# vitskvara/VBMatrixFactorization.jl

Hardware: AMD Instinct MI355X
Metric: VB iterations/sec (higher is better)
Workload: dtype bf16

## Files before the change

vbmatrixfactorization.jl_amd/csrc/gram_kernels.hpp:

```cpp
#pragma once
#include "common.hpp"
#include "ctrl_kernels.hpp"
#include "post_kernels.hpp"

namespace vbmf {

#ifndef GRAM_CHUNK
#define GRAM_CHUNK 256
#endif
constexpr int GRAM_PLANES = 5;
constexpr long long GRAM_G_NT_BYTES = 240LL << 20;

__device__ __forceinline__ unsigned pack_bf2(unsigned short lo, unsigned short hi) { return (unsigned)lo | ((unsigned)hi << 16); }

__global__ __launch_bounds__(256) void gram_build_kernel(const uint4* __restrict__ Y1, int XT, int KS, float* __restrict__ Gt,
                                                         int GT) {
    const int P = blockIdx.y, Q = blockIdx.x;
    if (P > Q) return;
    const int lane = threadIdx.x & 63, w = threadIdx.x >> 6;
    const int p0 = 4 * P + 2 * (w >> 1), q0 = 4 * Q + 2 * (w & 1);
    const long long KT = 2LL * GT;
    double g64[2][2][16];
#pragma unroll
    for (int a = 0; a < 2; ++a)
// ... 155 lines not shown
    for (int mb = 0; mb < GW_KS; ++mb) {
        const long long m = row0 + 16 * mb + c;
        f64x4 acc = {0.0, 0.0, 0.0, 0.0};
#pragma unroll
        for (int s = 0; s < NS; ++s) {
            const float4 a = m < M ? *reinterpret_cast<const float4*>(A32 + m * HP + 16 * s + 4 * q) : make_float4(0.f, 0.f, 0.f, 0.f);
            acc = __builtin_amdgcn_mfma_f64_16x16x4f64((double)a.x, sb[s][0], acc, 0, 0, 0);
            acc = __builtin_amdgcn_mfma_f64_16x16x4f64((double)a.y, sb[s][1], acc, 0, 0, 0);
            acc = __builtin_amdgcn_mfma_f64_16x16x4f64((double)a.z, sb[s][2], acc, 0, 0, 0);
            acc = __builtin_amdgcn_mfma_f64_16x16x4f64((double)a.w, sb[s][3], acc, 0, 0, 0);
        }
#pragma unroll
        for (int r = 0; r < 4; ++r) sW[16 * mb + q + 4 * r][16 * cb + c] = (float)acc[r];
    }
    __syncthreads();
    const long long plane = (long long)KT * NH * 64;
    for (int it = threadIdx.x; it < GW_KS * NHC * 64; it += NT) {
        const int jj = it / (NHC * 64), htl = (it / 64) % NHC, ln = it & 63;
        const int half = ln >> 5, hl = 32 * htl + (ln & 31), h = col0 + hl, ht = blockIdx.y * NHC + htl;
        const long long j = (long long)blockIdx.x * GW_KS + jj;
        if (j >= KT) continue;
        unsigned short wp[3][8], dp[2][8];
#pragma unroll
        for (int e = 0; e < 8; ++e) {
            const long long m = 16 * j + 8 * half + e;
            const float wv = sW[16 * jj + 8 * half + e][hl];
            const float dv = (float)((double)wv - (double)Wold[m * HP + h]);
            Wnew[m * HP + h] = wv;
            wp[0][e] = f2bf(wv);
            float res = wv - bf2f(wp[0][e]);
            wp[1][e] = f2bf(res);
            res -= bf2f(wp[1][e]);
            wp[2][e] = f2bf(res);
            dp[0][e] = f2bf(dv);
            dp[1][e] = f2bf(dv - bf2f(dp[0][e]));
        }
        const long long o = (j * NH + ht) * 64 + ln;
#pragma unroll
        for (int p = 0; p < 3; ++p)
            Wt[p * plane + o] = make_uint4(pack_bf2(wp[p][0], wp[p][1]), pack_bf2(wp[p][2], wp[p][3]), pack_bf2(wp[p][4], wp[p][5]),
                                           pack_bf2(wp[p][6], wp[p][7]));
#pragma unroll
        for (int p = 0; p < 2; ++p)
            Wt[(3 + p) * plane + o] = make_uint4(pack_bf2(dp[p][0], dp[p][1]), pack_bf2(dp[p][2], dp[p][3]), pack_bf2(dp[p][4], dp[p][5]),
                                                 pack_bf2(dp[p][6], dp[p][7]));
    }
}

__device__ __forceinline__ float sub_f32(float a, float b) {
    float r;
    asm("v_sub_f32 %0, %1, %2" : "=v"(r) : "v"(a), "v"(b));
    return r;
}
__device__ __forceinline__ unsigned cvt_pk_bf16(float lo, float hi) {
    typedef __attribute__((ext_vector_type(2))) float f32x2v;
    typedef __attribute__((ext_vector_type(2))) __bf16 bf16x2v;
    const f32x2v v = {lo, hi};
    return __builtin_bit_cast(unsigned, __builtin_convertvector(v, bf16x2v));
}
__device__ __forceinline__ void split3_frag(const f32x4& x0, const f32x4& x1, u32x4v& g0, u32x4v& g1, u32x4v& g2) {
    const float v[8] = {x0.x, x0.y, x0.z, x0.w, x1.x, x1.y, x1.z, x1.w};
#pragma unroll
    for (int e = 0; e < 4; ++e) {
        float a = v[2 * e], b = v[2 * e + 1];
        const unsigned p0 = cvt_pk_bf16(a, b);
        a = sub_f32(a, bitsf(p0 << 16));
        b = sub_f32(b, bitsf(p0 & 0xffff0000u));
        const unsigned p1 = cvt_pk_bf16(a, b);
        a = sub_f32(a, bitsf(p1 << 16));
        b = sub_f32(b, bitsf(p1 & 0xffff0000u));
        g0[e] = p0;
        g1[e] = p1;
        g2[e] = cvt_pk_bf16(a, b);
    }
}

__device__ __forceinline__ f32x16 mfma_bf(const u32x4v& a, const u32x4v& b, const f32x16& c) {
    return __builtin_amdgcn_mfma_f32_32x32x16_bf16(__builtin_bit_cast(bf16x8, a), __builtin_bit_cast(bf16x8, b), c, 0, 0, 0);
}

#ifndef VBMF_GRAMPROD_PROBE
#define VBMF_GRAMPROD_PROBE 0
#endif
template <int NH>
struct GramProd {
    static constexpr int NW = 8;
    static constexpr int THREADS = 64 * NW;
    static constexpr int TPG = 16 / NH;
    static constexpr int NXW = TPG >= NW ? TPG / NW : 1;
    static constexpr int HS = TPG >= NW ? 1 : NW / TPG;
    static constexpr int NHW = NH / HS;
    static constexpr int CH = NH == 2 ? 4 : 2;
    static constexpr int D = 4;
    static constexpr int U = CH;
    static constexpr int NP = GRAM_PLANES * CH * NH;
    static constexpr int PPW = (NP + NW - 1) / NW;
    static constexpr int GL = 2 * NXW;
    static constexpr int GQ = VBMF_GRAMPROD_PROBE == 2 ? 0 : GL;
    static constexpr int PLANE_BYTES = 2 * NP * 1024;
    static constexpr int RING_BYTES = NW * D * GL * 1024;
    static constexpr int LDS_BYTES = PLANE_BYTES + RING_BYTES;
    static_assert(NXW * (NW / HS) == TPG && NHW * HS == NH, "gram_prod geometry");
    static_assert(LDS_BYTES <= 160 * 1024, "gram_prod LDS");
    static constexpr int g_wait(int u) {
        int n = (D - 1) * GQ;
        for (int d = 1; d < D; ++d) n += ((u + CH * D - d) % CH == 0) ? PPW : 0;
        return n;
    }
};
template <int NH, int NHT = NH>
__global__ __launch_bounds__(GramProd<NH>::THREADS) void gram_prod_kernel(const float4* __restrict__ Gt, const uint4* __restrict__ Wt,
                                                                          float* __restrict__ Out, int GT, int XT1, int sps, int nrg,
                                                                          long long n, long long slab_floats,
                                                                          const int* __restrict__ stop) {
    using C = GramProd<NH>;
    constexpr int NW = C::NW, NXW = C::NXW, NHW = C::NHW, D = C::D, CH = C::CH, U = C::U, NP = C::NP, PPW = C::PPW, GL = C::GL;
    extern __shared__ __attribute__((aligned(1024))) unsigned char gram_lds[];
    if (*stop) return;
    const int lane = threadIdx.x & 63;
    const int w = __builtin_amdgcn_readfirstlane(threadIdx.x >> 6);
    const int rg = blockIdx.x % nrg, s = blockIdx.x / nrg;
    const int KT = 2 * GT;
    const int j0 = s * sps, j1 = min(j0 + sps, KT), nk = j1 - j0;
    const int pt0 = rg * C::TPG + (w % (C::TPG / NXW)) * NXW;
    const int h0 = (w / (C::TPG / NXW)) * NHW;
    const int hg0 = NHT == NH ? 0 : (int)blockIdx.y * NH;
    const long long plane = (long long)KT * NHT * 64;
    f32x16 accP[NXW][NHW], accQ[NXW][NHW];
#pragma unroll
    for (int i = 0; i < NXW; ++i)
#pragma unroll
        for (int h = 0; h < NHW; ++h)
#pragma unroll
            for (int r = 0; r < 16; ++r) { accP[i][h][r] = 0.f; accQ[i][h][r] = 0.f; }
    __amdgpu_buffer_rsrc_t gr[NXW];
#pragma unroll
    for (int i = 0; i < NXW; ++i)
        gr[i] = __builtin_amdgcn_make_buffer_rsrc((void*)(Gt + (long long)(pt0 + i) * KT * 128), 0,
                                                  VBMF_GRAMPROD_PROBE == 1 ? 0u : (unsigned)KT * 2048u, 0x00020000);
    const __amdgpu_buffer_rsrc_t wr = __builtin_amdgcn_make_buffer_rsrc((void*)Wt, 0, (unsigned)(GRAM_PLANES * plane * 16), 0x00020000);
    const int voff = lane * 16;
    unsigned char* const ring = gram_lds + C::PLANE_BYTES + w * (D * GL * 1024);
    const bool g_nt = !(NH == 4 && NHT == 4) && (long long)GT * GT * 4096 > GRAM_G_NT_BYTES;
    auto load_g = [&](int slot, int t) __attribute__((always_inline)) {
        const int so = VBMF_GRAMPROD_PROBE == 3 ? 0 : min(j0 + t, j1 - 1) * 2048;
        if (g_nt) {
#pragma unroll
            for (int i = 0; i < NXW; ++i) {
                lds_dma_piece_nt(gr[i], ring + (slot * GL + 2 * i) * 1024, voff, so);
                lds_dma_piece_nt(gr[i], ring + (slot * GL + 2 * i + 1) * 1024, voff, so + 1024);
            }
        } else {
#pragma unroll
            for (int i = 0; i < NXW; ++i) {
                lds_dma_piece(gr[i], ring + (slot * GL + 2 * i) * 1024, voff, so);
                lds_dma_piece(gr[i], ring + (slot * GL + 2 * i + 1) * 1024, voff, so + 1024);
            }
        }
    };
    auto load_planes = [&](int cc, int t) __attribute__((always_inline)) {
#pragma unroll
        for (int v = 0; v < PPW; ++v) {
            const int x = min(w + NW * v, NP - 1);
            const int q = x / (CH * NH), r = x % (CH * NH);
            const int j = min(j0 + t + r / NH, j1 - 1);
            lds_dma_piece(wr, gram_lds + (cc * NP + x) * 1024, voff, (int)(q * plane + ((long long)j * NHT + hg0 + r % NH) * 64) * 16);
        }
    };
#pragma unroll
    for (int d = 0; d < D; ++d) {
        if ((d + CH * D - D) % CH == 0) load_planes(0, 0);
        load_g(d, d);
    }
    asm volatile("s_waitcnt vmcnt(%0)" ::"n"(CH * GL) : "memory");
    __builtin_amdgcn_s_barrier();
    asm volatile("" ::: "memory");
    u32x4v wf[GRAM_PLANES][NHW], g[NXW][3];
    auto mma = [&]() __attribute__((always_inline)) {
#pragma unroll
        for (int i = 0; i < NXW; ++i) {
#pragma unroll
            for (int h = 0; h < NHW; ++h) {
                f32x16 a = accP[i][h];
                a = mfma_bf(wf[2][h], g[i][0], a);
                a = mfma_bf(wf[1][h], g[i][1], a);
                a = mfma_bf(wf[0][h], g[i][2], a);
                a = mfma_bf(wf[1][h], g[i][0], a);
                a = mfma_bf(wf[0][h], g[i][1], a);
                accP[i][h] = mfma_bf(wf[0][h], g[i][0], a);
                f32x16 d = accQ[i][h];
                d = mfma_bf(wf[4][h], g[i][0], d);
                d = mfma_bf(wf[3][h], g[i][1], d);
                accQ[i][h] = mfma_bf(wf[3][h], g[i][0], d);
            }
        }
    };
    int slot = 0;
    auto body = [&](int t0, bool tail) __attribute__((always_inline)) {
#pragma unroll
        for (int u = 0; u < U; ++u) {
            const int t = t0 + u, kk = u % CH;
            const int cc = (t / CH) & 1;
            const bool live = !tail || t < nk;
            asm volatile("s_waitcnt vmcnt(%0)" ::"n"(C::g_wait(u)) : "memory");
            if (live) {
                const unsigned char* gs = ring + slot * (GL * 1024) + lane * 32;
                f32x4 x[NXW][2];
#pragma unroll
                for (int i = 0; i < NXW; ++i) {
                    x[i][0] = *reinterpret_cast<const f32x4*>(gs + i * 2048);
                    x[i][1] = *reinterpret_cast<const f32x4*>(gs + i * 2048 + 16);
                }
                const unsigned char* pl = gram_lds + (cc * NP + kk * NH + h0) * 1024 + lane * 16;
#pragma unroll
                for (int q = 0; q < GRAM_PLANES; ++q)
#pragma unroll
                    for (int h = 0; h < NHW; ++h) wf[q][h] = *reinterpret_cast<const u32x4v*>(pl + (q * CH * NH + h) * 1024);
#pragma unroll
                for (int i = 0; i < NXW; ++i) split3_frag(x[i][0], x[i][1], g[i][0], g[i][1], g[i][2]);
            }
            __builtin_amdgcn_sched_barrier(0);
            if (kk == 0) load_planes(cc ^ 1, t + CH);
            if (VBMF_GRAMPROD_PROBE != 2) load_g(slot, t + D);
            slot = slot + 1 == D ? 0 : slot + 1;
            __builtin_amdgcn_sched_barrier(0);
            if (live) mma();
            if (kk == CH - 1) {
                asm volatile("s_waitcnt vmcnt(%0) lgkmcnt(0)" ::"n"(CH * C::GQ) : "memory");
                __builtin_amdgcn_s_barrier();
                asm volatile("" ::: "memory");
            }
        }
    };
    int t0 = 0;
    for (; t0 + U <= nk; t0 += U) body(t0, false);
    if (t0 < nk) body(t0, true);
    asm volatile("s_waitcnt vmcnt(0)" ::: "memory");
    float4* oP = reinterpret_cast<float4*>(Out + (long long)s * slab_floats);
    float4* oQ = reinterpret_cast<float4*>(Out + (long long)s * slab_floats + n);
#pragma unroll
    for (int i = 0; i < NXW; ++i) {
        const int p = pt0 + i;
        if (p >= XT1) continue;
#pragma unroll
        for (int h = 0; h < NHW; ++h) {
            const long long o = (((long long)p * NHT + hg0 + h0 + h) * 64 + lane) * 4;
            const f32x16 a = accP[i][h], d = accQ[i][h];
#pragma unroll
            for (int q = 0; q < 4; ++q) {
                oP[o + q] = float4{a[4 * q], a[4 * q + 1], a[4 * q + 2], a[4 * q + 3]};
                oQ[o + q] = float4{d[4 * q], d[4 * q + 1], d[4 * q + 2], d[4 * q + 3]};
            }
        }
    }
}

template <int HP>
struct GPart {
    static constexpr int V = HP / 16, S = 8 / V, NH = HP / 32;
    static constexpr int NT = 512, SD = 8;
    static constexpr int PPT = HP == 128 ? 2 : 3;
    static constexpr int ROWS = PPT * NT * 4 / HP;
    static constexpr int NSTEP = ROWS / 4 / S;
    static constexpr int BUF = ROWS * HP;
    static constexpr int SU = V == 8 ? 2 : 4;
    static_assert(NSTEP % SU == 0 && (ROWS / 4) % S == 0 && ROWS % 16 == 0, "gram_tail geometry");
    static_assert((S - 1) * V * V * 64 * 32 <= 2 * BUF * 4, "gram_tail: the subset fold reuses the block buffers");
};
template <int HP>
__device__ __forceinline__ int gpart_index(int a, int b) {
    constexpr int V = GPart<HP>::V;
    const int tw = a % V, i = a / V, t = b % V, c = b / V;
    return ((((tw * V + t) * 4 + (i >> 2)) << 6) + 16 * (i & 3) + c);
}
__device__ __forceinline__ void add4(float4& s, const float4& v) { s.x += v.x; s.y += v.y; s.z += v.z; s.w += v.w; }
struct GTailRound { float4 a0, a1, a2, a3, a4, a5, a6, a7; };
__device__ __forceinline__ void gtail_load(GTailRound& v, const __amdgpu_buffer_rsrc_t (&r)[8], int voff, int cnt) {
    const auto ld = [&](int u) __attribute__((always_inline)) {
        return __builtin_bit_cast(float4, __builtin_amdgcn_raw_buffer_load_b128(r[u], voff, 0, 0));
    };
    switch (cnt) {
        default: v.a7 = ld(7); [[fallthrough]];
        case 7: v.a6 = ld(6); [[fallthrough]];
        case 6: v.a5 = ld(5); [[fallthrough]];
        case 5: v.a4 = ld(4); [[fallthrough]];
        case 4: v.a3 = ld(3); [[fallthrough]];
        case 3: v.a2 = ld(2); [[fallthrough]];
        case 2: v.a1 = ld(1); [[fallthrough]];
        case 1: v.a0 = ld(0);
    }
}
template <bool FIRST>
__device__ __forceinline__ float4 gtail_sum(const GTailRound& v, float4 f, int cnt) {
    if (FIRST) f = v.a0;
    else add4(f, v.a0);
    if (cnt > 1) add4(f, v.a1);
    if (cnt > 2) add4(f, v.a2);
    if (cnt > 3) add4(f, v.a3);
    if (cnt > 4) add4(f, v.a4);
    if (cnt > 5) add4(f, v.a5);
    if (cnt > 6) add4(f, v.a6);
    if (cnt > 7) add4(f, v.a7);
    return f;
}
template <int HP, int HPT>
struct GPartBlk {
    static constexpr int NQ = HPT / HP;
    static constexpr long long STRIDE = 2LL * HPT * HPT + (NQ == 1 ? 1 : NQ);
};
template <int HP, int HPT = HP>
__global__ __launch_bounds__(512) void gram_tail_kernel(const float* slabs, int nslab, long long slab_floats, float* PQ, long long n,
                                                        long long Mp1, const float* __restrict__ Wn, const float* __restrict__ Wo,
                                                        const float* __restrict__ A32, long long M, int rpc, int nchunk,
                                                        double* __restrict__ part, const int* __restrict__ stop) {
    using C = GPart<HP>;
    constexpr int V = C::V, S = C::S, NH = C::NH, PPT = C::PPT, SD = C::SD, ROWS = C::ROWS, NSTEP = C::NSTEP, SU = C::SU;
    constexpr int NQ = GPartBlk<HP, HPT>::NQ, NHT = HPT / 32;
    constexpr bool BLK = NQ > 1;
    constexpr long long STRIDE = GPartBlk<HP, HPT>::STRIDE;
// ... 215 lines not shown
```

vbmatrixfactorization.jl_amd/csrc/vbmf_hip.hip:

```cpp
#include "../../include/vbmf_hip.h"

#include <hip/hip_runtime.h>
#include <rccl/rccl.h>

#include <algorithm>
#include <chrono>
#include <cmath>
#include <cstdio>
#include <cstring>
#include <string>
#include <thread>
#include <type_traits>
#include <vector>

#include "common.hpp"
#include "ctx_cache.hpp"
#include "ctx_mem.hpp"
#include "ctrl_kernels.hpp"
#include "post_kernels.hpp"
#include "rng.hpp"
#include "sparse_kernels.hpp"
#include "stream_gemm.hpp"
#include "tile_kernels.hpp"
#include "prep_kernels.hpp"
// ... 767 lines not shown
        }
        TRY(side_join(c));
        if (fused_gram(c)) TRY(launch_post_gram(c, 0, c->Pred));
        else if (c->P_frag) TRY(launch_post_frag(c, 0, c->Pred));
        else TRY(launch_post(c, 0, c->Pred, 1));
    } else {
        TRY(side_join(c));
        if (fused_gram(c)) TRY(launch_post_gram(c, 0, c->P));
        else if (c->P_frag) TRY(launch_post_frag(c, 0, c->P));
        else TRY(launch_post(c, 0, c->P, 1));
    }
    if (!fused_gram(c)) TRY(launch_gram(c, 0, c->A32, nullptr, true));
    c->cache.A_moved_basic();
    return VBMF_OK;
}

static int fold_Q_slabs(vbmf_ctx* c) {
    if (c->d2.nsplit <= 1) return VBMF_OK;
    const long long n = (long long)c->Hp * c->d2.XT * 32;
    hipLaunchKernelGGL(slab_sum_kernel, dim3(grid_for(n / 4, 256, 2048)), dim3(256), 0, c->stream, c->Q, c->d2.nsplit, n, c->Q, n,
                       c->ints + I_STOP, SideCopy{});
    HIPCHK(c, hipGetLastError());
    return VBMF_OK;
}

static int do_update_B(vbmf_ctx* c, bool keep_sigma = false) {
    TRY(ensure_gram_A(c));
    const bool epi = fused_gram(c) && !c->narrow && c->d2.nsplit == 1 && (c->d2.XT / nxw_of(c->NH) + 3) / 4 <= c->gslab_cap;
    if (epi) {
        int nslab = 0;
        if (fused_ctrl(c)) {
            TRY(launch_stream(c, 1, CTRL_COV_B | CTRL_EIG_BOLD, true, &nslab));
        } else {
            if (!keep_sigma) TRY(launch_ctrl_cov(c, 1));
            TRY(launch_stream(c, 1, 0, true, &nslab));
        }
        TRY(gram_reduce_tail(c, 1, true, c->ntr, true, nslab));
        c->bcur ^= 1;
        c->cache.B_moved_basic();
        return VBMF_OK;
    }
    const bool fragq = fused_gram(c) || c->d2.nsplit == 1;
    if (fused_ctrl(c)) {
        TRY(launch_stream(c, 1, CTRL_COV_B | CTRL_EIG_BOLD, false, nullptr, fragq));
    } else if (side_overlap(c)) {
        TRY(side_fork(c));
        TRY(launch_ctrl_cov(c, 1));
        TRY(side_end(c));
        TRY(launch_stream(c, 1, 0, false, nullptr, fragq));
    } else {
        if (!keep_sigma) TRY(launch_ctrl_cov(c, 1));
        TRY(launch_stream(c, 1, 0, false, nullptr, fragq));
    }
    TRY(fold_Q_slabs(c));
    TRY(side_join(c));
    if (fused_gram(c)) {
        TRY(launch_post_gram(c, 1, c->Q));
    } else {
        if (fragq) TRY(launch_post_frag(c));
        else TRY(launch_post(c, 1, c->Q, 1));
        TRY(launch_gram(c, 1, c->B32[c->bcur ^ 1], c->B32[c->bcur], true, c->ntr));
    }
    c->bcur ^= 1;
    c->cache.B_moved_basic();
    return VBMF_OK;
}

static bool gram_form_on(const vbmf_ctx* c) {
    return c->gram_form == VBMF_GRAM_FORM_ON || (c->gram_form == VBMF_GRAM_FORM_DEFAULT && c->gram_env == 3);
}
static bool gram_structural(const vbmf_ctx* c) {
    return !c->diagvar && !c->dual && !c->trial && !c->full_cov && !sharded(c) && c->o.nranks == 1 && c->o.y_dtype == VBMF_Y_BF16 &&
           c->mode == MODE_BF16X2 && (c->Hp <= 128 || (c->Hp == 256 && c->sparse && gram_form_on(c)));
}
static bool gram_eligible(const vbmf_ctx* c) {
    if (c->gram_form == VBMF_GRAM_FORM_OFF || !gram_structural(c)) return false;
    if (gram_form_on(c)) return true;
    if (c->gram_env == 0) return false;
    if (c->gram_env == 2 || (c->gram_env == 1 && !c->sparse)) return true;
    return c->L >= 4 * c->M && (double)c->L * (double)c->M >= 134217728.0;
}

static int gram_prod_nh(const vbmf_ctx* c) { return c->NH == 8 ? 4 : c->NH; }

static int gram_prepare(vbmf_ctx* c) {
    if (!c->Gt) {
        c->GT = (int)rup(c->d1.XT, 16);
        const int KT = 2 * c->GT;
        const int nhp = gram_prod_nh(c);
        c->g_nrg = c->GT / (16 / nhp);
        c->g_nsplit = std::max(1, std::min(KT / 8, NUM_CU / std::max(1, c->g_nrg)));
        if (c->NH != nhp) {
            const int w = c->g_nrg * (c->NH / nhp), smax = std::max(1, std::min(KT / 8, 4));
            int best = 1;
            for (int s = 2; s <= smax; ++s)
                if ((int64_t)cdiv(w * s, NUM_CU) * best < (int64_t)cdiv(w * best, NUM_CU) * s) best = s;
            c->g_nsplit = best;
        }
        c->g_sps = cdiv(KT, c->g_nsplit);
        c->g_nsplit = cdiv(KT, c->g_sps);
        const int64_t Mp1 = (int64_t)c->d1.XT * 32;
        c->g_nchunk = (int)std::max<int64_t>(1, std::min<int64_t>(c->Hp == 256 ? 32 : (c->Hp == 128 ? 64 : 128), cdiv(c->M, 64)));
        c->g_rpc = (int)rup(cdiv(c->M, c->g_nchunk), 16);
        c->g_nchunk = cdiv(c->M, c->g_rpc);
        const size_t n = (size_t)c->Hp * Mp1;
        const size_t wrows = (size_t)32 * c->GT;
        const size_t group = c->mem.mark();
        auto alloc = [&](auto*& slot, size_t bytes) -> int {
            int e = c->mem.acquire(slot, bytes);
            if (e == 0) e = (int)hipMemsetAsync(slot, 0, bytes, c->stream);
            return e;
        };
        int e = alloc(c->Gt, (size_t)c->GT * KT * 64 * 8 * 4);
        if (e == 0) e = alloc(c->W32g[0], wrows * c->Hp * 4);
        if (e == 0) e = alloc(c->W32g[1], wrows * c->Hp * 4);
        if (e == 0) e = alloc(c->Wt, (size_t)GRAM_PLANES * KT * c->NH * 64 * 16);
        if (e == 0) e = alloc(c->gPQ, 2 * n * 4);
        if (e == 0 && c->g_nsplit > 1) e = alloc(c->gslabs, (size_t)c->g_nsplit * 2 * n * 4);
        if (e == 0) e = alloc(c->g_part, (size_t)c->g_nchunk * (2 * (size_t)c->Hp * c->Hp + 2) * 8);
        if (e == 0) e = alloc(c->gsave, (2 * (size_t)c->Hp * c->Hp + 8) * 8);
        if (e != 0) {
            c->mem.rollback(group);
            FAIL(c, VBMF_ERR_HIP, "Gram-form sweep: device allocation failed (%s)", mem_errstr(e));
        }
        c->cache.G_buffers_new();
    }
    if (c->cache.G()) return VBMF_OK;
    hipEvent_t a, b;
    HIPCHK(c, hipEventCreate(&a));
    HIPCHK(c, hipEventCreate(&b));
    hipEventRecord(a, c->stream);
    const int NB = c->GT / 4;
    hipLaunchKernelGGL(gram_build_kernel, dim3(NB, NB), dim3(256), 0, c->stream, c->Y1, c->d1.XT, c->d1.KS, c->Gt, c->GT);
    const hipError_t le = hipGetLastError();
    hipEventRecord(b, c->stream);
    const hipError_t se = hipEventSynchronize(b);
    float ms = 0.f;
    hipEventElapsedTime(&ms, a, b);
    hipEventDestroy(a);
    hipEventDestroy(b);
    HIPCHK(c, le);
    HIPCHK(c, se);
    c->gram_build_ms = ms;
    c->cache.G_built();
    return VBMF_OK;
}

static int gram_product(vbmf_ctx* c, bool partials) {
    const int* stop = c->ints + I_STOP;
    const int KT = 2 * c->GT;
    const int64_t Mp1 = (int64_t)c->d1.XT * 32;
    const long long n = (long long)c->Hp * Mp1;
    const float* Wo = c->W32g[c->wcur];
    float* Wn = c->W32g[c->wcur ^ 1];
    const dim3 wg(cdiv(KT, GW_KS));
    const bool ok = dispatch<32, 64, 128, 256>(c->Hp, [&](auto hp) {
        constexpr int HPT = decltype(hp)::value, HPc = HPT == 256 ? 128 : HPT;
        if constexpr (HPT == 256)
            hipLaunchKernelGGL((gram_w_cols_kernel<256, 2>), dim3(wg.x, 2), dim3(512), 0, c->stream, c->A32, c->SB32, Wo, Wn, c->Wt, (long long)c->M, KT, stop);
        else
            hipLaunchKernelGGL((gram_w_kernel<HPT>), wg, dim3(HPT * 4), 0, c->stream, c->A32, c->SB32, Wo, Wn, c->Wt, (long long)c->M, KT, stop);
        float* out = c->g_nsplit > 1 ? c->gslabs : c->gPQ;
        const dim3 grid(c->g_nrg * c->g_nsplit, c->NH / gram_prod_nh(c));
        prof_begin(c, 0);
        {
            constexpr int NHT = HPT / 32, NHc = NHT == 8 ? 4 : NHT;
            hipLaunchKernelGGL((gram_prod_kernel<NHc, NHT>), grid, dim3(GramProd<NHc>::THREADS), GramProd<NHc>::LDS_BYTES, c->stream,
                               reinterpret_cast<const float4*>(c->Gt), c->Wt, out, c->GT, c->d1.XT, c->g_sps, c->g_nrg, n, 2 * n, stop);
        }
        prof_end(c);
        if (!partials) {
            if (c->g_nsplit > 1)
                hipLaunchKernelGGL(slab_sum_kernel, dim3(grid_for(2 * n / 4, 256, 2048)), dim3(256), 0, c->stream, c->gslabs, c->g_nsplit, 2 * n,
                                   c->gPQ, 2 * n, stop, SideCopy{});
            return;
        }
        const dim3 tg((HPT == 256 ? 8 : 2) * c->g_nchunk);
        hipLaunchKernelGGL((gram_tail_kernel<HPc, HPT>), tg, dim3(512), 0, c->stream, out, c->g_nsplit, 2 * n, c->gPQ, n, (long long)Mp1, Wn, Wo,
                           c->A32, (long long)c->M, c->g_rpc, c->g_nchunk, c->g_part, stop);
        const dim3 rg(cdiv(2 * (int64_t)c->Hp * c->Hp + 1, GRED_E));
        hipLaunchKernelGGL((gram_part_reduce_kernel<HPc, HPT>), rg, dim3(256), 0, c->stream, c->g_part, c->g_nchunk, c->st, c->lay, stop);
    });
    if (!ok) FAIL(c, VBMF_ERR_INVALID, "internal: the Gram-form sweep covers Hp <= 256");
    HIPCHK(c, hipGetLastError());
    return VBMF_OK;
}

static int launch_chain(vbmf_ctx* c, int mode, float* S32) {
    if (c->H > 128) FAIL(c, VBMF_ERR_INVALID, "internal: the stand-alone control chain covers H <= 128");
    const CtrlArgs ca = ctrl_args(c, mode, S32);
    const int parts = (mode & CTRL_EIG_AHEAD) ? 3 : ((mode & (CTRL_PREV_END | CTRL_EIG_BOLD)) ? 2 : 1);
    ctrl_tier(c->H, [&](auto r, auto t) {
        constexpr int R = decltype(r)::value;
        const int nthr = (mode & (CTRL_PREV_END | CTRL_EIG_AHEAD | CTRL_EIG_BOLD)) ? eig_wide_launch(R, ca.spectral) : 256;
        if constexpr (decltype(t)::value == 16)
            hipLaunchKernelGGL((ctrl_chain_kernel<R>), dim3(parts), dim3(nthr), ctrl_lds_bytes_r(R), c->stream, ca);
    });
    HIPCHK(c, hipGetLastError());
    return VBMF_OK;
}

static int gram_sweep(vbmf_ctx* c) {
    TRY(launch_chain(c, CTRL_COV_A | CTRL_EIG_AHEAD | (c->tail_pending ? CTRL_PREV_END : 0), c->SA32));
    if (c->tail_pending) ++c->ends_enqueued;
    c->tail_pending = false;
    c->P_frag = true;
    if (fused_gram(c)) TRY(launch_post_gram(c, 0, c->gPQ));
    else {
        TRY(launch_post_frag(c, 0, c->gPQ));
        TRY(launch_gram(c, 0, c->A32, nullptr, true));
    }
    TRY(launch_chain(c, CTRL_COMMIT_A | CTRL_COV_B, c->SB32));
    TRY(gram_product(c, true));
    c->wcur ^= 1;
    c->cache.gram_sweep_done_basic();
    return VBMF_OK;
}

static int prepare_trYBA(vbmf_ctx* c, int* flag) {
    *flag = 0;
    if (c->cache.tr()) return VBMF_OK;
    double* dst = c->st + c->lay.GX();
    HIPCHK(c, hipMemsetAsync(dst, 0, sizeof(double), c->stream));
    if (c->cache.P()) {
        const float* In = (sharded(c) || c->d1.nsplit > 1) ? c->Pred : c->P;
        const int ns = 1;
        const long long ld = (long long)c->d1.XT * 32;
        const int g = grid_for(c->M, 256, 1024);
        hipLaunchKernelGGL(dot_kernel, dim3(g), dim3(256), 0, c->stream, In, ld, ns,
                           (long long)c->Hp * ld, c->A32, c->Hp, (long long)c->M, c->ypart, c->P_frag ? c->NH : 0);
        hipLaunchKernelGGL(sum_partials_kernel, dim3(1), dim3(256), 0, c->stream, c->ypart, g, dst);
    } else {
        TRY(launch_stream(c, 1));
        const long long ld = (long long)c->d2.XT * 32;
        const int g = grid_for(c->L, 256, 1024);
        hipLaunchKernelGGL(dot_kernel, dim3(g), dim3(256), 0, c->stream, c->Q, ld, c->d2.nsplit,
                           (long long)c->Hp * ld, c->B32[c->bcur], c->Hp, (long long)c->L, c->ypart, 0);
        hipLaunchKernelGGL(sum_partials_kernel, dim3(1), dim3(256), 0, c->stream, c->ypart, g, dst);
        if (sharded(c)) TRY(allreduce_sum(c, dst, 1, true));
    }
    HIPCHK(c, hipGetLastError());
    c->cache.tr_made();
    return VBMF_OK;
}

static double d_resolution(const vbmf_ctx* c) { return c->mode == MODE_F32 ? 2e-6 : (c->mode == MODE_BF16X2 ? 1e-5 : 4e-3); }
static void run_note_eps(vbmf_ctx* c, int64_t niter, double eps, int64_t done, double d) {
    c->err.clear();
    if (done >= niter && eps > 0.0 && d > eps && eps < d_resolution(c)) {
        char b[400];
        snprintf(b, sizeof b, "note: all %lld sweeps ran and d = %.3g is still above eps = %.3g, which is below what d resolves in this "
// ... 356 lines not shown
    const int nchunk = std::max(std::max(cdiv(c->d1.XT, gram_tiles_per_chunk(c, 0)), cdiv(c->d2.XT, gram_tiles_per_chunk(c, 1))),
                                std::max(cdiv(c->d1.XT, c->tiles_per_chunk), cdiv(c->d2.XT, c->tiles_per_chunk)));
    {
        const int epi_blocks = (c->NH <= 2) ? std::min(1024, (c->d2.XT / nxw_of(c->NH) + 3) / 4) : 0;
        c->gslab_cap = std::max(256, epi_blocks);
        c->gslab_bytes = std::max((size_t)nchunk * 2 * c->Hp * c->Hp * 4, (size_t)c->gslab_cap * 2 * 3 * 1024 * 4);
        ALLOC(c->gslab, c->gslab_bytes);
    }
    ALLOC(c->st, (size_t)c->lay.total() * 8);
    ALLOC(c->gtmp, ((size_t)2 * c->Hp * c->Hp + 8) * 8);
    c->trpart_cap = 4 * std::max(c->gslab_cap, (c->d2.XT + 3) / 4 + 1);
    ALLOC(c->trpart, (size_t)c->trpart_cap * 8);
    ALLOC(c->ypart, (size_t)16384 * 8);
    ALLOC(c->ints, 32 * sizeof(int));
    ALLOC(c->mask, (size_t)c->Mp);
    if (c->sparse) {
        ALLOC(c->dS32, (size_t)c->Mp * c->Hp * 4);
        ALLOC(c->CA32, (size_t)c->Mp * c->Hp * 4);
        ALLOC(c->beta32, (size_t)c->Mp * c->Hp * 4);
        ALLOC(c->vtab, (size_t)c->Hp * 8);
    }
    if (c->dual) {
        c->gpart_blocks = grid_for((int64_t)c->M * c->Hp);
        ALLOC(c->gpart, (size_t)c->gpart_blocks * 6 * 8);
    }
    if (c->diagvar) {
        ALLOC(c->sigv, (size_t)c->Lp * 8);
        ALLOC(c->zetav, (size_t)c->Lp * 8);
        ALLOC(c->yrow, (size_t)c->Lp * 8);
        ALLOC(c->hpart, (size_t)cdiv(c->Lp, 256) * 8 + 64);
        ALLOC(c->hmean, 2 * 8);
        ALLOC(c->vsq, (size_t)c->Hp * 8);
        ALLOC(c->sig32, (size_t)c->Lp * 4);
        ALLOC(c->G32, (size_t)c->Hp * c->Hp * 4);
        ALLOC(c->FBs_alloc, (c->nFB + flead) * 16);
        c->FBs = c->FBs_alloc + flead;
    }
#undef ALLOC
    if (hipHostMalloc((void**)&c->ints_host, 16 * sizeof(int)) != hipSuccess ||
        hipHostMalloc((void**)&c->scal_host, 32 * sizeof(double)) != hipSuccess) {
        c->err = "pinned alloc failed"; return bail(VBMF_ERR_HIP);
    }
    if (hipHostMalloc((void**)&c->loopw, 16 * sizeof(int), hipHostMallocMapped | hipHostMallocCoherent) != hipSuccess ||
        hipHostGetDevicePointer((void**)&c->loopw_dev, c->loopw, 0) != hipSuccess) {
        c->err = "host-mapped alloc failed"; return bail(VBMF_ERR_HIP);
    }
    memset(c->loopw, 0, 16 * sizeof(int));
    if (hipStreamCreateWithFlags(&c->stream, hipStreamNonBlocking) != hipSuccess) { c->err = "stream create failed"; return bail(VBMF_ERR_HIP); }
    if (hipStreamCreateWithFlags(&c->side, hipStreamNonBlocking) != hipSuccess ||
        hipEventCreateWithFlags(&c->ev_main, hipEventDisableTiming) != hipSuccess ||
        hipEventCreateWithFlags(&c->ev_side, hipEventDisableTiming) != hipSuccess) { c->err = "side stream create failed"; return bail(VBMF_ERR_HIP); }
    c->lds_limit = 160 * 1024 - 16384;
    {
        const int lim = c->lds_limit, vb = (int)vbls_lds_bytes(4), fb = (int)FITB_LDS_CAP;
        const struct { const void* kernel; int bytes; int nh; } big_lds[] = {
            {(const void*)eig_kernel<8>, lim, 0},
            {(const void*)ctrl_cov_kernel<8, 16>, lim, 0},
            {(const void*)ctrl_chain_kernel<8>, lim, 0},
            {(const void*)sparse_cov_b_kernel<8, 16>, lim, 0},
            {(const void*)ctrl_cov_kernel<8, 32>, lim, 0}, {(const void*)sparse_cov_b_kernel<8, 32>, lim, 0},
            {(const void*)sparse_update_a_full256_kernel, lim, 0},
            {(const void*)sparse_update_a_full_wave_kernel<1, 8>, (int)full_a_wave_lds_bytes(1, 8), 0},
            {(const void*)sparse_update_a_full_wave_kernel<2, 8>, (int)full_a_wave_lds_bytes(2, 8), 0},
            {(const void*)sparse_update_a_full_wave_kernel<4, 4>, (int)full_a_wave_lds_bytes(4, 4), 0},
            {(const void*)vbls_loop_kernel<4>, vb, 0}, {(const void*)vbls_batch_kernel<4>, vb, 0},
            {(const void*)sparse_batch_kernel<4, true>, (int)SBATCH_LDS_BIG, 0},
            {(const void*)fit_batch_kernel<1, false>, fb, 0}, {(const void*)fit_batch_kernel<1, true>, fb, 0},
            {(const void*)fit_batch_kernel<2, false>, fb, 0}, {(const void*)fit_batch_kernel<2, true>, fb, 0},
            {(const void*)fit_batch_kernel<1, false, true>, fb, 0}, {(const void*)fit_batch_kernel<1, true, true>, fb, 0},
            {(const void*)fit_batch_kernel<2, false, true>, fb, 0}, {(const void*)fit_batch_kernel<2, true, true>, fb, 0},
            {(const void*)fit_batch_kernel<1, false, true, true>, fb, 0}, {(const void*)fit_batch_kernel<1, true, true, true>, fb, 0},
            {(const void*)fit_batch_kernel<2, false, true, true>, fb, 0}, {(const void*)fit_batch_kernel<2, true, true, true>, fb, 0},
            {(const void*)fit_cols_kernel<1, false, false>, fb, 0}, {(const void*)fit_cols_kernel<1, true, false>, fb, 0},
            {(const void*)fit_cols_kernel<2, false, false>, fb, 0}, {(const void*)fit_cols_kernel<2, true, false>, fb, 0},
            {(const void*)fit_cols_kernel<1, false, true>, fb, 0}, {(const void*)fit_cols_kernel<1, true, true>, fb, 0},
            {(const void*)fit_cols_kernel<2, false, true>, fb, 0}, {(const void*)fit_cols_kernel<2, true, true>, fb, 0},
            {(const void*)fit_fold_kernel<1, false>, fb, 0}, {(const void*)fit_fold_kernel<2, false>, fb, 0},
            {(const void*)fit_fold_kernel<1, true>, fb, 0}, {(const void*)fit_fold_kernel<2, true>, fb, 0},
            {(const void*)fit_basic_kernel<1>, fb, 0}, {(const void*)fit_basic_kernel<2>, fb, 0},
            {(const void*)fit_basic_gram_kernel<1>, fb, 0}, {(const void*)fit_basic_gram_kernel<2>, fb, 0},
            {(const void*)stream_lds8_kernel<4, StreamCfg<4>::Rc, false>, LDS8_BYTES, 4},
            {(const void*)stream_lds8_kernel<4, StreamCfg<4>::Rc, true>, LDS8_BYTES, 4},
            {(const void*)stream_lds8_kernel<8, 0, false>, LDS8_BYTES, 8}, {(const void*)stream_lds8_kernel<8, 0, true>, LDS8_BYTES, 8},
            {(const void*)gram_prod_kernel<1>, GramProd<1>::LDS_BYTES, 1},
            {(const void*)gram_prod_kernel<2>, GramProd<2>::LDS_BYTES, 2},
            {(const void*)gram_prod_kernel<4>, GramProd<4>::LDS_BYTES, 4},
            {(const void*)gram_prod_kernel<4, 8>, GramProd<4>::LDS_BYTES, 8},
        };
        hipError_t e = hipSuccess;
        for (const auto& r : big_lds)
            if (e == hipSuccess && (r.nh == 0 || r.nh == c->NH))
                e = hipFuncSetAttribute(r.kernel, hipFuncAttributeMaxDynamicSharedMemorySize, r.bytes);
        if (e == hipSuccess && c->NH == 4) {
            using Cfg = StreamCfg<4>;
            dispatch<MODE_F32, MODE_BF16, MODE_BF16X2>(c->mode, [&](auto md) {
                e = hipFuncSetAttribute((const void*)stream_gemm_kernel<decltype(md)::value, 4, Cfg::NXWc, Cfg::DYc, Cfg::DFc, Cfg::Rc>,
                                        hipFuncAttributeMaxDynamicSharedMemorySize, c->lds_limit);
            });
        }
        if (e != hipSuccess) { c->err = "hipFuncSetAttribute(MaxDynamicSharedMemorySize) failed"; return bail(VBMF_ERR_HIP); }
    }
    if (hipDeviceSynchronize() != hipSuccess) { c->err = "hipDeviceSynchronize failed"; return bail(VBMF_ERR_HIP); }
    *out = c;
    return VBMF_OK;
}

}

struct TileRange { int xa, xb, ka, kb; };
template <class Src>
static int launch_tiles(vbmf_ctx* c, const Src& src, TileRange r1, TileRange r2, double* sumsq) {
    const int64_t n1 = (int64_t)(r1.xb - r1.xa) * (r1.kb - r1.ka) * 64, n2 = (int64_t)(r2.xb - r2.xa) * (r2.kb - r2.ka) * 64;
    dispatch<MODE_F32, MODE_BF16>(ymode_of(c->mode), [&](auto ym) {
        constexpr int TM = decltype(ym)::value;
        hipLaunchKernelGGL((tile_y_kernel<TM, false, Src>), dim3(grid_for(n1, 256, 16384)), dim3(256), 0, c->stream, c->Y1,
                           src, r1.xa, r1.xb, r1.ka, r1.kb, c->d1.KS, (double*)nullptr);
        const int g2 = grid_for(n2, 256, 16384);
        hipLaunchKernelGGL((tile_y_kernel<TM, true, Src>), dim3(g2), dim3(256), 0, c->stream, c->Y2,
                           src, r2.xa, r2.xb, r2.ka, r2.kb, c->d2.KS, sumsq ? c->ypart : nullptr);
        if (sumsq) hipLaunchKernelGGL(sum_partials_kernel, dim3(1), dim3(256), 0, c->stream, c->ypart, g2, sumsq);
    });
    HIPCHK(c, hipGetLastError());
    return VBMF_OK;
}

template <class Src>
static int build_tiles(vbmf_ctx* c, const Src& src, int64_t m0, int64_t m1, double* sumsq) {
    const int xt0 = (int)(m0 / 32), xt1 = (m1 >= c->M) ? c->d1.XT : (int)(m1 / 32);
    const int ks0 = (int)(m0 / c->kstep), ks1 = (m1 >= c->M) ? c->d2.KS : (int)(m1 / c->kstep);
    return launch_tiles(c, src, TileRange{xt0, xt1, 0, c->d1.KS}, TileRange{0, c->d2.XT, ks0, ks1}, sumsq);
}

template <class Src>
static int build_tiles_rows(vbmf_ctx* c, const Src& src, int64_t l0, int64_t l1, double* sumsq) {
    const int ks0 = (int)(l0 / c->kstep), ks1 = (l1 >= c->L) ? c->d1.KS : (int)(l1 / c->kstep);
    const int xt0 = (int)(l0 / 32), xt1 = (l1 >= c->L) ? c->d2.XT : (int)(l1 / 32);
    return launch_tiles(c, src, TileRange{0, c->d1.XT, ks0, ks1}, TileRange{xt0, xt1, 0, c->d2.KS}, sumsq);
}

template <class T>
static int launch_tile_pair(vbmf_ctx* c, const T* dev, int64_t l0, int64_t l1, int64_t rs, int64_t cs, double* sumsq) {
    const bool last = l1 >= c->L;
    const int ks = c->kstep;
    const int k1a = (int)(l0 / ks), k1b = last ? c->d1.KS : (int)(l1 / ks);
    const int x2a = (int)(l0 / 32), x2b = last ? c->d2.XT : (int)(l1 / 32);
    const int64_t l_end = last ? std::max<int64_t>((int64_t)c->d2.XT * 32, (int64_t)c->d1.KS * ks) : l1;
    const int64_t m_end = std::max<int64_t>((int64_t)c->d1.XT * 32, (int64_t)c->d2.KS * ks);
    PairGeom g;
    uint4 *outA, *outB;
    if (cs == 1) {
        g.ss = rs; g.s_org = l0; g.u_org = 0; g.s_lo = l0; g.s_hi = l1; g.u_lo = 0; g.u_hi = c->M; g.s0 = l0; g.u0 = 0;
        g.ns = (int)cdiv(l_end - l0, 32); g.nu = (int)cdiv(m_end, PAIR_U);
        g.xa0 = x2a; g.xa1 = x2b; g.ka0 = 0; g.ka1 = c->d2.KS; g.KSA = c->d2.KS; outA = c->Y2;
        g.xb0 = 0; g.xb1 = c->d1.XT; g.kb0 = k1a; g.kb1 = k1b; g.KSB = c->d1.KS; outB = c->Y1;
    } else {
        g.ss = cs; g.s_org = 0; g.u_org = l0; g.s_lo = 0; g.s_hi = c->M; g.u_lo = l0; g.u_hi = l1; g.s0 = 0; g.u0 = l0;
        g.ns = (int)cdiv(m_end, 32); g.nu = (int)cdiv(l_end - l0, PAIR_U);
        g.xa0 = 0; g.xa1 = c->d1.XT; g.ka0 = k1a; g.ka1 = k1b; g.KSA = c->d1.KS; outA = c->Y1;
        g.xb0 = x2a; g.xb1 = x2b; g.kb0 = 0; g.kb1 = c->d2.KS; g.KSB = c->d2.KS; outB = c->Y2;
    }
    const int grid = (int)std::min<int64_t>((int64_t)g.ns * g.nu, 16384);
    dispatch<MODE_F32, MODE_BF16>(ymode_of(c->mode), [&](auto ym) {
        constexpr int TM = decltype(ym)::value;
        hipLaunchKernelGGL((tile_pair_kernel<TM, T>), dim3(grid), dim3(256), 0, c->stream, outA, outB, dev, g, c->ypart);
        hipLaunchKernelGGL(sum_partials_kernel, dim3(1), dim3(256), 0, c->stream, c->ypart, grid, sumsq);
    });
    HIPCHK(c, hipGetLastError());
    return VBMF_OK;
}

// ... 1736 lines not shown
```

Measured before the change: 4948.

## Software-pipeline gram_prod: double-buffer fragments and interleave split with MFMA

Restructures the gram_prod main loop into a software-pipelined form. The next chunk's G fragments are split into bf16 pieces while the current chunk's MFMAs run, using two register sets, and weight-plane LDS reads are prefetched a step ahead. It also makes the non-temporal G load choice a template parameter instead of a runtime branch, and hoists the plane-address math out of the loop. The goal is to hide LDS-read and split VALU latency behind matrix work, at the cost of more registers and possible spills or occupancy loss.

After: 4970, median of 6. No clear change (+0.5%).

```diff
diff --git a/vbmatrixfactorization.jl_amd/csrc/gram_kernels.hpp b/vbmatrixfactorization.jl_amd/csrc/gram_kernels.hpp
--- a/vbmatrixfactorization.jl_amd/csrc/gram_kernels.hpp
+++ b/vbmatrixfactorization.jl_amd/csrc/gram_kernels.hpp
@@ -261,6 +261,9 @@
 #ifndef VBMF_GRAMPROD_PROBE
 #define VBMF_GRAMPROD_PROBE 0
 #endif
+#ifndef VBMF_GRAMPROD_SWP
+#define VBMF_GRAMPROD_SWP 7
+#endif
 template <int NH>
 struct GramProd {
     static constexpr int NW = 8;
@@ -272,6 +275,7 @@
     static constexpr int CH = NH == 2 ? 4 : 2;
     static constexpr int D = 4;
     static constexpr int U = CH;
+    static constexpr bool SWP = VBMF_GRAMPROD_PROBE == 0 && ((VBMF_GRAMPROD_SWP >> (NH >> 1)) & 1);
     static constexpr int NP = GRAM_PLANES * CH * NH;
     static constexpr int PPW = (NP + NW - 1) / NW;
     static constexpr int GL = 2 * NXW;
@@ -286,8 +290,14 @@
         for (int d = 1; d < D; ++d) n += ((u + CH * D - d) % CH == 0) ? PPW : 0;
         return n;
     }
+    static constexpr int g_wait0() {
+        int n = (D - 1) * GL;
+        for (int s = 2; s <= D; ++s) n += ((CH * D - s) % CH == 0) ? PPW : 0;
+        return n;
+    }
+    static_assert(!SWP || (U % 2 == 0 && D >= CH && CH >= 2), "gram_prod pipelined loop: two register sets, chunk 0 issued by a prologue body");
 };
-template <int NH, int NHT = NH>
+template <int NH, int NHT = NH, bool G_NT = false>
 __global__ __launch_bounds__(GramProd<NH>::THREADS) void gram_prod_kernel(const float4* __restrict__ Gt, const uint4* __restrict__ Wt,
                                                                           float* __restrict__ Out, int GT, int XT1, int sps, int nrg,
                                                                           long long n, long long slab_floats,
@@ -320,100 +330,188 @@
     const __amdgpu_buffer_rsrc_t wr = __builtin_amdgcn_make_buffer_rsrc((void*)Wt, 0, (unsigned)(GRAM_PLANES * plane * 16), 0x00020000);
     const int voff = lane * 16;
     unsigned char* const ring = gram_lds + C::PLANE_BYTES + w * (D * GL * 1024);
-    const bool g_nt = !(NH == 4 && NHT == 4) && (long long)GT * GT * 4096 > GRAM_G_NT_BYTES;
     auto load_g = [&](int slot, int t) __attribute__((always_inline)) {
         const int so = VBMF_GRAMPROD_PROBE == 3 ? 0 : min(j0 + t, j1 - 1) * 2048;
-        if (g_nt) {
-#pragma unroll
-            for (int i = 0; i < NXW; ++i) {
+#pragma unroll
+        for (int i = 0; i < NXW; ++i) {
+            if constexpr (G_NT) {
                 lds_dma_piece_nt(gr[i], ring + (slot * GL + 2 * i) * 1024, voff, so);
                 lds_dma_piece_nt(gr[i], ring + (slot * GL + 2 * i + 1) * 1024, voff, so + 1024);
-            }
-        } else {
-#pragma unroll
-            for (int i = 0; i < NXW; ++i) {
+            } else {
                 lds_dma_piece(gr[i], ring + (slot * GL + 2 * i) * 1024, voff, so);
                 lds_dma_piece(gr[i], ring + (slot * GL + 2 * i + 1) * 1024, voff, so + 1024);
             }
         }
     };
+    int pl_lds[PPW], pl_off[PPW], pl_kk[PPW];
+#pragma unroll
+    for (int v = 0; v < PPW; ++v) {
+        const int x = min(w + NW * v, NP - 1);
+        const int q = x / (CH * NH), r = x % (CH * NH);
+        pl_lds[v] = x * 1024;
+        pl_off[v] = (int)(q * plane + (long long)(hg0 + r % NH) * 64) * 16;
+        pl_kk[v] = r / NH;
+    }
     auto load_planes = [&](int cc, int t) __attribute__((always_inline)) {
 #pragma unroll
-        for (int v = 0; v < PPW; ++v) {
-            const int x = min(w + NW * v, NP - 1);
-            const int q = x / (CH * NH), r = x % (CH * NH);
-            const int j = min(j0 + t + r / NH, j1 - 1);
-            lds_dma_piece(wr, gram_lds + (cc * NP + x) * 1024, voff, (int)(q * plane + ((long long)j * NHT + hg0 + r % NH) * 64) * 16);
-        }
-    };
-#pragma unroll
-    for (int d = 0; d < D; ++d) {
-        if ((d + CH * D - D) % CH == 0) load_planes(0, 0);
-        load_g(d, d);
-    }
-    asm volatile("s_waitcnt vmcnt(%0)" ::"n"(CH * GL) : "memory");
-    __builtin_amdgcn_s_barrier();
-    asm volatile("" ::: "memory");
-    u32x4v wf[GRAM_PLANES][NHW], g[NXW][3];
-    auto mma = [&]() __attribute__((always_inline)) {
+        for (int v = 0; v < PPW; ++v)
+            lds_dma_piece(wr, gram_lds + cc * (NP * 1024) + pl_lds[v], voff, pl_off[v] + min(j0 + t + pl_kk[v], j1 - 1) * (NHT * 1024));
+    };
+    constexpr bool WF2 = C::SWP && NHW == 1;
+    u32x4v wf[WF2 ? 2 : 1][GRAM_PLANES][NHW], g[C::SWP ? 2 : 1][NXW][3];
+    f32x4 x[NXW][2];
+    auto read_g = [&](int sl) __attribute__((always_inline)) {
+        const unsigned char* gs = ring + sl * (GL * 1024) + lane * 32;
 #pragma unroll
         for (int i = 0; i < NXW; ++i) {
-#pragma unroll
-            for (int h = 0; h < NHW; ++h) {
-                f32x16 a = accP[i][h];
-                a = mfma_bf(wf[2][h], g[i][0], a);
-                a = mfma_bf(wf[1][h], g[i][1], a);
-                a = mfma_bf(wf[0][h], g[i][2], a);
-                a = mfma_bf(wf[1][h], g[i][0], a);
-                a = mfma_bf(wf[0][h], g[i][1], a);
-                accP[i][h] = mfma_bf(wf[0][h], g[i][0], a);
-                f32x16 d = accQ[i][h];
-                d = mfma_bf(wf[4][h], g[i][0], d);
-                d = mfma_bf(wf[3][h], g[i][1], d);
-                accQ[i][h] = mfma_bf(wf[3][h], g[i][0], d);
+            x[i][0] = *reinterpret_cast<const f32x4*>(gs + i * 2048);
+            x[i][1] = *reinterpret_cast<const f32x4*>(gs + i * 2048 + 16);
+        }
+    };
+    auto read_planes_h = [&](int b, int h, int cc, int kk) __attribute__((always_inline)) {
+        const unsigned char* pl = gram_lds + (cc * NP + kk * NH + h0 + h) * 1024 + lane * 16;
+#pragma unroll
+        for (int q = 0; q < GRAM_PLANES; ++q) wf[b][q][h] = *reinterpret_cast<const u32x4v*>(pl + (q * CH * NH) * 1024);
+    };
+    auto read_planes = [&](int b, int cc, int kk) __attribute__((always_inline)) {
+        const unsigned char* pl = gram_lds + (cc * NP + kk * NH + h0) * 1024 + lane * 16;
+#pragma unroll
+        for (int q = 0; q < GRAM_PLANES; ++q)
+#pragma unroll
+            for (int h = 0; h < NHW; ++h) wf[b][q][h] = *reinterpret_cast<const u32x4v*>(pl + (q * CH * NH + h) * 1024);
+    };
+    auto split = [&](int b) __attribute__((always_inline)) {
+#pragma unroll
+        for (int i = 0; i < NXW; ++i) split3_frag(x[i][0], x[i][1], g[b][i][0], g[b][i][1], g[b][i][2]);
+    };
+    auto mfma_step = [&](int bw, int bg, int i, int h, int j) __attribute__((always_inline)) {
+        constexpr int WP[9] = {2, 1, 0, 1, 0, 0, 4, 3, 3}, GP[9] = {0, 1, 2, 0, 1, 0, 0, 1, 0};
+        if (j < 6) accP[i][h] = mfma_bf(wf[bw][WP[j]][h], g[bg][i][GP[j]], accP[i][h]);
+        else accQ[i][h] = mfma_bf(wf[bw][WP[j]][h], g[bg][i][GP[j]], accQ[i][h]);
+    };
+    auto mma = [&](int b) __attribute__((always_inline)) {
+#pragma unroll
+        for (int i = 0; i < NXW; ++i)
+#pragma unroll
+            for (int h = 0; h < NHW; ++h)
+#pragma unroll
+                for (int j = 0; j < 9; ++j) mfma_step(b, b, i, h, j);
+    };
+    int t0 = 0;
+    if constexpr (C::SWP) {
+        load_g(0, 0);
+#pragma unroll
+        for (int d = 1; d < D; ++d) {
+            if ((CH * D + d - 1 - D) % CH == 0) load_planes(0, 0);
+            load_g(d, d);
+        }
+        asm volatile("s_waitcnt vmcnt(%0)" ::"n"(C::g_wait0()) : "memory");
+        read_g(0);
+        split(0);
+        __builtin_amdgcn_sched_barrier(0);
+        load_g(0, D);
+        asm volatile("s_waitcnt vmcnt(%0)" ::"n"(CH * GL) : "memory");
+        __builtin_amdgcn_s_barrier();
+        asm volatile("" ::: "memory");
+        int slot = 1 % D;
+        constexpr int NM = 9 * NXW * NHW, NCH = 8 * NXW;
+        float ra[NXW][4], rb[NXW][4];
+        auto split_piece = [&](int b, int c) __attribute__((always_inline)) {
+            const int i = c / 8, e = (c % 8) / 2;
+            if (c % 2 == 0) {
+                const float a = x[i][e / 2][2 * (e % 2)], bb = x[i][e / 2][2 * (e % 2) + 1];
+                const unsigned p0 = cvt_pk_bf16(a, bb);
+                ra[i][e] = sub_f32(a, bitsf(p0 << 16));
+                rb[i][e] = sub_f32(bb, bitsf(p0 & 0xffff0000u));
+                g[b][i][0][e] = p0;
+            } else {
+                const unsigned p1 = cvt_pk_bf16(ra[i][e], rb[i][e]);
+                const float a = sub_f32(ra[i][e], bitsf(p1 << 16)), bb = sub_f32(rb[i][e], bitsf(p1 & 0xffff0000u));
+                g[b][i][1][e] = p1;
+                g[b][i][2][e] = cvt_pk_bf16(a, bb);
             }
-        }
-    };
-    int slot = 0;
-    auto body = [&](int t0, bool tail) __attribute__((always_inline)) {
-#pragma unroll
-        for (int u = 0; u < U; ++u) {
-            const int t = t0 + u, kk = u % CH;
-            const int cc = (t / CH) & 1;
-            const bool live = !tail || t < nk;
-            asm volatile("s_waitcnt vmcnt(%0)" ::"n"(C::g_wait(u)) : "memory");
-            if (live) {
-                const unsigned char* gs = ring + slot * (GL * 1024) + lane * 32;
-                f32x4 x[NXW][2];
-#pragma unroll
-                for (int i = 0; i < NXW; ++i) {
-                    x[i][0] = *reinterpret_cast<const f32x4*>(gs + i * 2048);
-                    x[i][1] = *reinterpret_cast<const f32x4*>(gs + i * 2048 + 16);
+        };
+        auto body = [&](int t0, bool tail) __attribute__((always_inline)) {
+#pragma unroll
+            for (int u = 0; u < U; ++u) {
+                const int t = t0 + u, kk = u % CH, bg = u & 1, bw = WF2 ? bg : 0;
+                const int cc = (t / CH) & 1;
+                const bool live = !tail || t < nk;
+                __builtin_amdgcn_sched_barrier(0);
+                if (kk == 0) {
+                    read_planes(bw, cc, 0);
+                } else if (!WF2) {
+#pragma unroll
+                    for (int h = 1; h < NHW; ++h) read_planes_h(0, h, cc, kk);
                 }
-                const unsigned char* pl = gram_lds + (cc * NP + kk * NH + h0) * 1024 + lane * 16;
-#pragma unroll
-                for (int q = 0; q < GRAM_PLANES; ++q)
-#pragma unroll
-                    for (int h = 0; h < NHW; ++h) wf[q][h] = *reinterpret_cast<const u32x4v*>(pl + (q * CH * NH + h) * 1024);
-#pragma unroll
-                for (int i = 0; i < NXW; ++i) split3_frag(x[i][0], x[i][1], g[i][0], g[i][1], g[i][2]);
+                asm volatile("s_waitcnt vmcnt(%0)" ::"n"(C::g_wait(u)) : "memory");
+                read_g(slot);
+                if (WF2 && kk != CH - 1) read_planes(bw ^ 1, cc, kk + 1);
+#pragma unroll
+                for (int m = 0; m < NM; ++m) {
+                    const int i = m / (9 * NHW), h = (m / 9) % NHW, j = m % 9;
+                    if (live) mfma_step(bw, bg, i, h, j);
+                    if (!WF2 && i == NXW - 1 && h == 0 && j == 8 && kk != CH - 1) read_planes_h(0, 0, cc, kk + 1);
+                    __builtin_amdgcn_sched_barrier(0);
+#pragma unroll
+                    for (int c = 0; c < NCH; ++c) {
+                        if (1 + c * (NM - 2) / NCH == m) {
+                            split_piece(bg ^ 1, c);
+                            __builtin_amdgcn_sched_barrier(0);
+                        }
+                    }
+                }
+                __builtin_amdgcn_sched_barrier(0);
+                if (kk == 0) load_planes(cc ^ 1, t + CH);
+                load_g(slot, t + 1 + D);
+                slot = slot + 1 == D ? 0 : slot + 1;
+                if (kk == CH - 1) {
+                    asm volatile("s_waitcnt vmcnt(%0) lgkmcnt(0)" ::"n"(CH * C::GQ) : "memory");
+                    __builtin_amdgcn_s_barrier();
+                    asm volatile("" ::: "memory");
+                }
             }
-            __builtin_amdgcn_sched_barrier(0);
-            if (kk == 0) load_planes(cc ^ 1, t + CH);
-            if (VBMF_GRAMPROD_PROBE != 2) load_g(slot, t + D);
-            slot = slot + 1 == D ? 0 : slot + 1;
-            __builtin_amdgcn_sched_barrier(0);
-            if (live) mma();
-            if (kk == CH - 1) {
-                asm volatile("s_waitcnt vmcnt(%0) lgkmcnt(0)" ::"n"(CH * C::GQ) : "memory");
-                __builtin_amdgcn_s_barrier();
-                asm volatile("" ::: "memory");
+        };
+        for (; t0 + U <= nk; t0 += U) body(t0, false);
+        if (t0 < nk) body(t0, true);
+    } else {
+#pragma unroll
+        for (int d = 0; d < D; ++d) {
+            if ((d + CH * D - D) % CH == 0) load_planes(0, 0);
+            load_g(d, d);
+        }
+        asm volatile("s_waitcnt vmcnt(%0)" ::"n"(CH * GL) : "memory");
+        __builtin_amdgcn_s_barrier();
+        asm volatile("" ::: "memory");
+        int slot = 0;
+        auto body = [&](int t0, bool tail) __attribute__((always_inline)) {
+#pragma unroll
+            for (int u = 0; u < U; ++u) {
+                const int t = t0 + u, kk = u % CH;
+                const int cc = (t / CH) & 1;
+                const bool live = !tail || t < nk;
+                asm volatile("s_waitcnt vmcnt(%0)" ::"n"(C::g_wait(u)) : "memory");
+                if (live) {
+                    read_g(slot);
+                    read_planes(0, cc, kk);
+                    split(0);
+                }
+                __builtin_amdgcn_sched_barrier(0);
+                if (kk == 0) load_planes(cc ^ 1, t + CH);
+                if (VBMF_GRAMPROD_PROBE != 2) load_g(slot, t + D);
+                slot = slot + 1 == D ? 0 : slot + 1;
+                __builtin_amdgcn_sched_barrier(0);
+                if (live) mma(0);
+                if (kk == CH - 1) {
+                    asm volatile("s_waitcnt vmcnt(%0) lgkmcnt(0)" ::"n"(CH * C::GQ) : "memory");
+                    __builtin_amdgcn_s_barrier();
+                    asm volatile("" ::: "memory");
+                }
             }
-        }
-    };
-    int t0 = 0;
-    for (; t0 + U <= nk; t0 += U) body(t0, false);
-    if (t0 < nk) body(t0, true);
+        };
+        for (; t0 + U <= nk; t0 += U) body(t0, false);
+        if (t0 < nk) body(t0, true);
+    }
     asm volatile("s_waitcnt vmcnt(0)" ::: "memory");
     float4* oP = reinterpret_cast<float4*>(Out + (long long)s * slab_floats);
     float4* oQ = reinterpret_cast<float4*>(Out + (long long)s * slab_floats + n);
diff --git a/vbmatrixfactorization.jl_amd/csrc/vbmf_hip.hip b/vbmatrixfactorization.jl_amd/csrc/vbmf_hip.hip
--- a/vbmatrixfactorization.jl_amd/csrc/vbmf_hip.hip
+++ b/vbmatrixfactorization.jl_amd/csrc/vbmf_hip.hip
@@ -873,6 +873,7 @@
 }
 
 static int gram_prod_nh(const vbmf_ctx* c) { return c->NH == 8 ? 4 : c->NH; }
+static bool gram_prod_g_nt(const vbmf_ctx* c) { return c->NH != 4 && (long long)c->GT * c->GT * 4096 > GRAM_G_NT_BYTES; }
 
 static int gram_prepare(vbmf_ctx* c) {
     if (!c->Gt) {
@@ -956,8 +957,13 @@
         prof_begin(c, 0);
         {
             constexpr int NHT = HPT / 32, NHc = NHT == 8 ? 4 : NHT;
-            hipLaunchKernelGGL((gram_prod_kernel<NHc, NHT>), grid, dim3(GramProd<NHc>::THREADS), GramProd<NHc>::LDS_BYTES, c->stream,
-                               reinterpret_cast<const float4*>(c->Gt), c->Wt, out, c->GT, c->d1.XT, c->g_sps, c->g_nrg, n, 2 * n, stop);
+            const auto launch = [&](auto nt) {
+                hipLaunchKernelGGL((gram_prod_kernel<NHc, NHT, decltype(nt)::value>), grid, dim3(GramProd<NHc>::THREADS), GramProd<NHc>::LDS_BYTES,
+                                   c->stream, reinterpret_cast<const float4*>(c->Gt), c->Wt, out, c->GT, c->d1.XT, c->g_sps, c->g_nrg, n, 2 * n, stop);
+            };
+            if constexpr (NHT == 4) launch(std::false_type{});
+            else if (gram_prod_g_nt(c)) launch(std::true_type{});
+            else launch(std::false_type{});
         }
         prof_end(c);
         if (!partials) {
@@ -1480,10 +1486,10 @@
             {(const void*)stream_lds8_kernel<4, StreamCfg<4>::Rc, false>, LDS8_BYTES, 4},
             {(const void*)stream_lds8_kernel<4, StreamCfg<4>::Rc, true>, LDS8_BYTES, 4},
             {(const void*)stream_lds8_kernel<8, 0, false>, LDS8_BYTES, 8}, {(const void*)stream_lds8_kernel<8, 0, true>, LDS8_BYTES, 8},
-            {(const void*)gram_prod_kernel<1>, GramProd<1>::LDS_BYTES, 1},
-            {(const void*)gram_prod_kernel<2>, GramProd<2>::LDS_BYTES, 2},
+            {(const void*)gram_prod_kernel<1>, GramProd<1>::LDS_BYTES, 1}, {(const void*)gram_prod_kernel<1, 1, true>, GramProd<1>::LDS_BYTES, 1},
+            {(const void*)gram_prod_kernel<2>, GramProd<2>::LDS_BYTES, 2}, {(const void*)gram_prod_kernel<2, 2, true>, GramProd<2>::LDS_BYTES, 2},
             {(const void*)gram_prod_kernel<4>, GramProd<4>::LDS_BYTES, 4},
-            {(const void*)gram_prod_kernel<4, 8>, GramProd<4>::LDS_BYTES, 8},
+            {(const void*)gram_prod_kernel<4, 8>, GramProd<4>::LDS_BYTES, 8}, {(const void*)gram_prod_kernel<4, 8, true>, GramProd<4>::LDS_BYTES, 8},
         };
         hipError_t e = hipSuccess;
         for (const auto& r : big_lds)
```
